# amcpherson/remixt

Hardware: AMD Instinct MI355X
Metric: EM iterations/sec (50k seg x 165 states) (higher is better)
Workload: dtype f64

## Files before the change

### include/remixt_amd.h

```cpp
#ifndef REMIXT_AMD_H
#define REMIXT_AMD_H

#include <stdint.h>

#ifdef __cplusplus
extern "C" {
#endif

#define RMX_OK 0
#define RMX_EVALUE 1
#define RMX_EASSERT 2
#define RMX_EDEVICE 3
#define RMX_EUNSUPPORTED 4
#define RMX_EARG 5

#define RMX_MAX_CLONES 4

typedef struct rmx_batch rmx_batch;

typedef struct rmx_problem {
    int32_t num_clones;
    int32_t num_segments;
    int32_t num_breakpoints;
    int32_t num_cn_states;
// ... 58 lines not shown
    RMX_OPT_SEARCH_MODE,
    RMX_OPT_ELL_DENSE,
    RMX_OPT_STRIP,
    RMX_OPT_CELL_CACHE,
    RMX_OPT_SPARSE_TRIAL,
    RMX_OPT_FB_DEBUG,
    RMX_OPT_PAIRWISE_KERNEL,
    RMX_OPT_PACE_SWEEPS,
    RMX_OPT_FB_WG_BUDGET,
    RMX_OPT_TRIAL_KERNEL,
    RMX_OPT_GRAD_KERNEL,
    RMX_OPT_STREAM_POOL,
    RMX_OPT_VITERBI_CLUSTER,
    RMX_OPT_TRACEBACK,
    RMX_OPT_LT_CLASSES,
    RMX_OPT_COUNT
};
int rmx_set_default_option(int32_t option_id, int32_t value);
int rmx_set_option(rmx_batch *b, int32_t option_id, int32_t value);
int rmx_get_option(rmx_batch *b, int32_t option_id, int32_t *value);

int rmx_set_param(rmx_batch *b, int32_t r, int32_t param_id, double value);
int rmx_get_param(rmx_batch *b, int32_t r, int32_t param_id, double *value);
int rmx_set_transition_model(rmx_batch *b, int32_t model);
int rmx_set_array(rmx_batch *b, int32_t r, int32_t array_id, const void *host_src);
int rmx_get_array(rmx_batch *b, int32_t r, int32_t array_id, void *host_dst);
int rmx_fetch_indicators(rmx_batch *b, int32_t r0, int32_t r1, const double **total, const double **allele);
int rmx_calculate_log_transmat(rmx_batch *b, int32_t r, double *dst);
int rmx_weighted_search(const double *p, int64_t n, const double *u, int32_t k, int64_t *out, int64_t *positive);
int rmx_weighted_sample_round(const double *w, int64_t n, int64_t stride, double norm, const double *u, int32_t k,
// ... 74 lines not shown
```

### remixt_amd/bpmodel.py

```python
import ctypes as C

import numpy as np

from . import _lib

_dp = C.POINTER(C.c_double)
_ip = C.POINTER(C.c_int64)
_i32p = C.POINTER(C.c_int32)

RMX_EVALUE, RMX_EASSERT, RMX_EDEVICE, RMX_EUNSUPPORTED, RMX_EARG = 1, 2, 3, 4, 5

MAX_CLONES = 4
PARAM_IDS = {
    'negbin_r_0': 0, 'negbin_r_1': 1, 'negbin_hdel_mu': 2, 'negbin_hdel_r_0': 3, 'negbin_hdel_r_1': 4,
    'betabin_M_0': 5, 'betabin_M_1': 6, 'betabin_loh_p': 7, 'betabin_loh_M_0': 8, 'betabin_loh_M_1': 9,
    'prior_outlier_total': 10, 'prior_outlier_allele': 11, 'divergence_weight': 12, 'hmm_log_norm_const': 13,
}
ARRAY_IDS = {
    'h': 0, 'p_breakpoint': 1, 'p_allele_swap': 2, 'p_outlier_total': 3, 'p_outlier_allele': 4,
    'posterior_marginals': 5, 'framelogprob': 6, 'total_likelihood_mask': 7, 'allele_likelihood_mask': 8,
    'log_transmat': 9, 'cached_log_transmat': 10, 'joint_posterior_marginals': 11, 'state_sequence': 12,
}
_WRITABLE = {'h', 'p_breakpoint', 'p_allele_swap', 'p_outlier_total', 'p_outlier_allele', 'posterior_marginals',
             'total_likelihood_mask', 'allele_likelihood_mask'}
_STATE_TABLES = {'cn_states_total': 0, 'num_alleles_subclonal': 1, 'is_hdel': 2, 'is_loh': 3}


OPTION_IDS = dict((n, i) for i, n in enumerate((
    'fb_kernel', 'fb_nv', 'fb_breakend_codes', 'fuse_sweeps', 'two_streams', 'viterbi_plain', 'search_mode', 'ell_dense', 'strip',
    'cell_cache', 'sparse_trial', 'fb_debug', 'pairwise_kernel', 'pace_sweeps', 'fb_wg_budget', 'trial_kernel', 'grad_kernel', 'stream_pool', 'viterbi_cluster', 'traceback', 'lt_classes')))


def set_default_option(name, value):
    lib = _lib.load()
    rc = lib.rmx_set_default_option(OPTION_IDS[name], int(value))
    if rc:
        _raise(lib, rc)


def last_error_restarts():
    lib = _lib.load()
    n = lib.rmx_last_error_restarts(None, 0)
    if n <= 0:
        return []
    buf = (C.c_int32 * n)()
# ... 791 lines not shown
```

### remixt_amd/csrc/rmx_api.hip

```cpp
#include <hip/hip_runtime.h>
#include <algorithm>
#include <cmath>
#include <limits>
#include <atomic>
#include <cstdio>
#include <cstring>
#include <functional>
#include <map>
#include <mutex>
#include <string>
#include <vector>
#include <chrono>
#include <cstdlib>
#include <condition_variable>
#include <memory>

#include "rmx_kernels.h"
#include "rmx_host.h"

static thread_local std::string g_err;
static thread_local std::vector<int32_t> g_err_restarts;
static int fail(int code, const std::string &msg) { g_err = msg; g_err_restarts.clear(); return code; }
static int fail_flagged(int code, const std::string &msg) { g_err = msg; return code; }
static inline long long now_ns() { return std::chrono::duration_cast<std::chrono::nanoseconds>(std::chrono::steady_clock::now().time_since_epoch()).count(); }
// ... 21 lines not shown
    StreamPool &p = g_stream_pool[dev & 15];
    std::lock_guard<std::mutex> lk(p.mu);
    std::vector<hipStream_t> &idle = p.idle[role];
    if (!idle.empty()) { *out = idle.front(); idle.erase(idle.begin()); return RMX_OK; }
    if (hipStreamCreateWithFlags(out, hipStreamNonBlocking) != hipSuccess) return RMX_EDEVICE;
    p.created[role]++;
    return RMX_OK;
}
static void pool_release(int dev, int role, hipStream_t s) {
    hipStreamSynchronize(s);
    StreamPool &p = g_stream_pool[dev & 15];
    std::lock_guard<std::mutex> lk(p.mu);
    p.idle[role].push_back(s);
}

static int g_opt_default[RMX_OPT_COUNT] = {0, 0, 1, 1, 1, 0, 5, 0, 1, 1, 1, 0, 0, 0, 0, 0, 0, 1, 0, 0, 1};
static std::mutex g_opt_mu;

struct rmx_batch {
    hipEvent_t ev_pace = nullptr;
    int opt[RMX_OPT_COUNT];
    int device = 0;
    hipStream_t stream = nullptr;
    hipStream_t stream2 = nullptr;
    hipEvent_t ev_fb = nullptr, ev_brk = nullptr;
    bool own_stream = false, pooled_stream = false, pooled_stream2 = false;
    Dev d{};
    int R = 0;
    std::vector<int64_t> cn_classes;
    std::vector<int32_t> seg_class, brk_idx, brk_orient, tclass, brk_slot, be_n;
    std::vector<int64_t> brk_states, is_telomere;
// ... 25 lines not shown
    int32_t *h_lists = nullptr;
    size_t h_lists_cap = 0;
    hipEvent_t ev_lists = nullptr;
    uint32_t *h_err = nullptr;
    int32_t *d_sample = nullptr;
    NmState *d_nm_state = nullptr;
    NmLayout nm_lay = {nullptr, nullptr, nullptr}; double *d_nm_partial = nullptr; size_t nm_partial_cap = 0;
    int32_t *d_msample = nullptr, *d_mcounts = nullptr;
    std::vector<int> msample_count;
    double *d_mpartial = nullptr; size_t mpartial_cap = 0;
    std::vector<std::vector<int64_t>> sample_cache; std::vector<int> sample_count;
    double *d_grid_out = nullptr;
    GradFlatLayout gf_lay = {nullptr, nullptr, nullptr, nullptr};
    std::vector<double> gf_sig;
    std::vector<long long> sample_epoch, sig_epoch;
    int32_t *gf_nblk_host = nullptr;
    bool gf_first = false;
    unsigned *d_done = nullptr;
    int32_t *d_rlist = nullptr, *d_counts = nullptr; RestartParams *d_rp_stage = nullptr; double *d_batch_out = nullptr;
    void *h_batch = nullptr;
    std::vector<int32_t> plain_list; int32_t *d_plain_list = nullptr; double *d_plain_jt = nullptr;
    int last_search_blocks = 0;
    unsigned *d_vflag = nullptr; int cluster_timeouts = 0;
    int last_viterbi_wgs = 1;
    int32_t *d_vit_special = nullptr; int n_vit_special = -1;
    double *h_elbo = nullptr; hipEvent_t ev_elbo = nullptr; bool elbo_pending = false, elbo_sync = false; int elbo_r0 = 0, elbo_r1 = 0;
    double *d_vrow = nullptr; size_t vrow_cap = 0;
    uint16_t *d_bp = nullptr; double *d_final = nullptr; int64_t *d_path = nullptr; double *d_logprob = nullptr;
    std::vector<int64_t> last_path; int vit_cap = 0; size_t bp_cap = 0;
    int16_t *d_samp = nullptr; size_t samp_cap = 0; uint64_t *d_seeds = nullptr; uint32_t *d_sflags = nullptr;
// ... 78 lines not shown
        return id == KID_FRAMELOGPROB || id == KID_FB || id == KID_MARGINALS || id == KID_PAIRWISE || id == KID_BRK_LUT ||
               id == KID_BRK_UPDATE || id == KID_OUTLIER_TOTAL || id == KID_OUTLIER_ALLELE || id == KID_ALLELE_SWAP;
    }
    ProfScope(rmx_batch *b_, int id_) : b(b_), id(id_) {
        on = b->prof == 1 || (b->prof == 2 && sweep_kernel(id));
        if (on) { a = get_event(b); e = get_event(b); hipEventRecord(a, b->stream); }
    }
    void restart(int id_) { id = id_; if (on) hipEventRecord(a, b->stream); }
    void cancel() { if (on) { b->ev_pool.push_back(a); b->ev_pool.push_back(e); on = false; } }
    ~ProfScope() {
        if (on) { hipEventRecord(e, b->stream); b->prof_pending.push_back({id, a, e}); if (b->prof_pending.size() > 8192) prof_collect(b); }
    }
};

static int translate_error(rmx_batch *b, int r, uint32_t v);
static int check_errors(rmx_batch *b, int r0, int r1) {
    uint32_t *e = b->h_err;
    HIPCHK(hipMemcpyAsync(e, b->d.err, sizeof(uint32_t) * b->R, hipMemcpyDeviceToHost, b->stream));
    HIPCHK(hipStreamSynchronize(b->stream));
    int first = -1;
    for (int r = r0; r < r1; r++) if (e[r]) { if (first < 0) { first = r; g_err_restarts.clear(); } g_err_restarts.push_back(r); }
    if (first < 0) return RMX_OK;
    HIPCHK(hipMemsetAsync(b->d.err + r0, 0, sizeof(uint32_t) * (size_t)(r1 - r0), b->stream));
    return translate_error(b, first, e[first]);
}
template <typename F> static int report_request_errors(rmx_batch *b, int n, const uint32_t *words, F restart_of) {
    int first = -1;
    for (int i = 0; i < n; i++) {
        if (!words[i]) continue;
        const int r = restart_of(i);
        if (first < 0) { first = i; g_err_restarts.clear(); }
        if (std::find(g_err_restarts.begin(), g_err_restarts.end(), r) == g_err_restarts.end()) {
            g_err_restarts.push_back(r);
// ... 850 lines not shown
    return RMX_OK;
}
int rmx_synchronize(rmx_batch *b) { BIND(b); HIPCHK(hipStreamSynchronize(b->stream)); return RMX_OK; }

int rmx_info(rmx_batch *b, int32_t what, int64_t *out) { BIND(b);
    switch (what) {
    case 0: *out = b->d.cn_max; break; case 1: *out = b->d.NC; break; case 2: *out = b->d.TC; break; case 3: *out = b->d.NBE; break;
    case 4: *out = b->d.SP; break; case 5: *out = b->fbv_rpt; break; case 6: *out = b->fbG.P; break; case 7: *out = b->fbG.NT; break;
    case 8: *out = b->fbG.BLK; break; case 9: *out = (int64_t)b->fbG_lds; break; case 10: *out = b->n_fast; break; case 11: *out = b->n_generic; break;
    case 60: *out = b->t_launch_ns; break; case 61: *out = b->t_wait_ns; break; case 62: *out = b->t_post_ns; break; case 63: *out = b->n_rounds; break;
    case 12: *out = b->last_fb_kernel; break; case 13: *out = b->last_fb_nv; break; case 14: *out = b->last_viterbi; break; case 15: *out = b->last_fb_nv_max; break;
    case 18: *out = b->last_viterbi_wgs; break; case 19: *out = b->last_traceback; break;
    case 64: *out = b->d.NT; break; case 65: *out = b->d.ltc ? 1 : 0; break;
    case 54: *out = b->cluster_timeouts; break;
    case 52: *out = b->last_search_blocks; break;
    case 16: { StreamPool &p_ = g_stream_pool[b->device & 15]; std::lock_guard<std::mutex> lk(p_.mu); *out = p_.created[0] + p_.created[1]; break; }
    case 17: { StreamPool &p_ = g_stream_pool[b->device & 15]; std::lock_guard<std::mutex> lk(p_.mu); *out = (int64_t)(p_.idle[0].size() + p_.idle[1].size()); break; }
    case 20: case 21: case 22: case 23: case 24: case 25: case 26: case 27: case 28: case 29: case 30: case 31: case 32: case 33: case 34: case 35: case 36: case 37: case 38: case 39:
    case 40: case 41: case 42: case 43: case 44: case 45: case 46: case 47: case 48: case 49: case 50: case 51:
        { if (!b->d_dbg) { *out = 0; break; } unsigned long long v[32]; HIPCHK(hipStreamSynchronize(b->stream)); HIPCHK(hipMemcpy(v, b->d_dbg, 256, hipMemcpyDeviceToHost)); *out = (int64_t)v[what - 20]; break; }
    default: return fail(RMX_EARG, "bad info id");
    }
    return RMX_OK;
}

static const int kParamComponents[RMX_P_HMM_LOG_NORM_CONST] = {CM_LT0, CM_LT1, CM_LT0 | CM_LT1, CM_LT0, CM_LT1, CM_LA0, CM_LA1, CM_LA0 | CM_LA1, CM_LA0, CM_LA1, 0, 0, 16};
int rmx_set_param(rmx_batch *b, int32_t r, int32_t id, double v) { BIND(b);
    if (r < 0 || r >= b->R || id < 0 || id >= RMX_P_HMM_LOG_NORM_CONST) return fail(RMX_EARG, "bad restart / param id");
    if (id == RMX_P_DIVERGENCE_WEIGHT) v = std::fabs(v);
    b->rp[r].p[id] = v; b->tables_dirty[r] = 1; b->ab_dirty[r] = 1;
// ... 604 lines not shown
    RANGE_CHECK();
    if (b->elbo_pending) return fail(RMX_EARG, "an ELBO is already pending: rmx_calculate_elbo_end first");
    const int nr = r1 - r0;
    if (!b->h_elbo) {
        HIPCHK(hipHostMalloc((void **)&b->h_elbo, ((size_t)b->R * 4 + (size_t)b->R) * 8, hipHostMallocDefault));
        HIPCHK(hipEventCreateWithFlags(&b->ev_elbo, hipEventDisableTiming));
    }
    bool mixed = false;
    for (int r = r0; r < r1; r++) mixed |= b->lt_valid[r] && b->lt_model[r] != b->cached_model[r];
    b->elbo_r0 = r0; b->elbo_r1 = r1; b->elbo_sync = mixed;
    b->elbo_pending = true;
    if (mixed) return RMX_OK;
    int rc = ensure_ab(b, r0, r1);
    if (rc) { b->elbo_pending = false; return rc; }
    { ProfScope ps(b, KID_ELBO_SEG); hipLaunchKernelGGL(k_elbo_seg, dim3(ELBO_BLOCKS, nr), dim3(256), 0, b->stream, b->d, r0, b->d_partial, b->d_be_e); }
    for (int r = r0; r < r1;) {
        int e = r + 1;
        while (e < r1 && b->plain_T_init[e] == b->plain_T_init[r]) e++;
        ProfScope ps(b, KID_ELBO_FINAL);
        hipLaunchKernelGGL(k_elbo_final, dim3(e - r), dim3(256), 0, b->stream, b->d, r, b->d_partial + (size_t)(r - r0) * ELBO_BLOCKS * 3,
                           b->d_be_e + (size_t)(r - r0) * b->d.NBE, ELBO_BLOCKS,
                           (const int *)b->d_lt_valid, b->plain_T_init[r], (const double *)nullptr, b->d_out4 + (size_t)(r - r0) * 4);
        r = e;
    }
    HIPCHK(hipGetLastError());
    HIPCHK(hipMemcpyAsync(b->h_elbo, b->d_out4, (size_t)nr * 32, hipMemcpyDeviceToHost, b->stream));
    HIPCHK(hipMemcpyAsync(b->h_elbo + (size_t)b->R * 4, b->d.err, sizeof(uint32_t) * b->R, hipMemcpyDeviceToHost, b->stream));
    HIPCHK(hipEventRecord(b->ev_elbo, b->stream));
    return RMX_OK;
}
int rmx_calculate_elbo_end(rmx_batch *b, double *out) { BIND(b);
    if (!b || !out) return fail(RMX_EARG, "bad argument");
    if (!b->elbo_pending) return fail(RMX_EARG, "no ELBO pending");
    b->elbo_pending = false;
    const int r0 = b->elbo_r0, r1 = b->elbo_r1;
    if (b->elbo_sync) return rmx_calculate_elbo(b, r0, r1, out);
    HIPCHK(hipEventSynchronize(b->ev_elbo));
    const uint32_t *e = reinterpret_cast<const uint32_t *>(b->h_elbo + (size_t)b->R * 4);
    int first = -1;
    for (int r = r0; r < r1; r++) if (e[r]) { if (first < 0) { first = r; g_err_restarts.clear(); } g_err_restarts.push_back(r); }
    if (first >= 0) {
        std::lock_guard<std::mutex> lk(b->mu);
// ... 113 lines not shown
        }
        HIPCHK(hipMemcpyAsync(hp, gout, (size_t)G * W * 8, hipMemcpyDeviceToHost, b->stream));
        if ((rc = finish_restart(b, r, eh))) return rc;
    }
    HIPCHK(hipEventSynchronize(b->done_ev[r]));
    if (*eh) { uint32_t v = *eh; std::lock_guard<std::mutex> lk(b->mu); HIPCHK(hipMemsetAsync(b->d.err + r, 0, sizeof(uint32_t), b->stream)); return translate_error(b, r, v); }
    for (int g = 0; g < G; g++) out[g] = hp[(size_t)g * W];
    return RMX_OK;
}

static bool gradflat_ready(rmx_batch *b, int nreq, const int32_t *restarts, const StageArgs &sa) {
    if (!b->gf_lay.upre) {
        const size_t R = (size_t)b->R;
        if (dalloc(b, &b->gf_lay.upre, R * (NM_MAX_SAMPLE + 1)) != RMX_OK || dalloc(b, &b->gf_lay.blk, R * (NM_MAX_SAMPLE + 2)) != RMX_OK ||
            dalloc(b, &b->gf_lay.nblk, R) != RMX_OK || dalloc(b, &b->gf_lay.k8, R * NM_MAX_SAMPLE * 8) != RMX_OK) { b->gf_lay.upre = nullptr; return false; }
        if (hipHostMalloc((void **)&b->gf_nblk_host, 16 * sizeof(int32_t), hipHostMallocDefault) != hipSuccess) { b->gf_lay.upre = nullptr; return false; }
    }
    std::vector<double> sig;
    sig.reserve((size_t)nreq * (3 + RMX_P_HMM_LOG_NORM_CONST));
    for (int i = 0; i < nreq; i++) {
        const int r = restarts[i];
        sig.push_back((double)r); sig.push_back((double)b->sample_epoch[r]); sig.push_back((double)b->sig_epoch[r]);
        for (int k = 0; k < RMX_P_HMM_LOG_NORM_CONST; k++) sig.push_back(sa.rp[i].p[k]);
    }
    if (sig == b->gf_sig) return true;
    hipLaunchKernelGGL(k_gradflat_setup, dim3(nreq), dim3(256), 0, b->stream, b->d, sa, (const int32_t *)b->d_sample, (const int32_t *)b->d_counts, b->gf_lay, b->gf_nblk_host);
    if (hipGetLastError() != hipSuccess) return false;
    b->gf_sig.swap(sig);
    b->gf_first = true;
    return true;
}
static int run_ell_batch(rmx_batch *b, int nreq, const int32_t *restarts, bool grad, double *out, int mask = CM_ALL) {
    const Dev &d = b->d;
    const long long t_in = now_ns();
    const int W = 1 + RMX_MAX_CLONES;
    const int nout = grad ? W : 1;
    int maxcnt = 0;
    const bool by_value = nreq <= 16;
    StageArgs sa;
    RestartParams *hs = by_value ? sa.rp : (RestartParams *)b->h_batch;
    int32_t *hl = by_value ? sa.rlist : (int32_t *)((char *)b->h_batch + (size_t)b->R * sizeof(RestartParams));
    for (int i = 0; i < nreq; i++) {
        const int r = restarts[i];
// ... 10 lines not shown
            ProfScope ps(b, KID_STATE_TABLES);
            hipLaunchKernelGGL(k_state_tables_list_v, dim3(d.C, nreq), dim3(256), 0, b->stream, b->d, sa, b->d_rlist, b->d_rp_stage);
        } else {
            HIPCHK(hipMemcpyAsync(b->d_rp_stage, hs, (size_t)nreq * sizeof(RestartParams), hipMemcpyHostToDevice, b->stream));
            HIPCHK(hipMemcpyAsync(b->d_rlist, hl, (size_t)nreq * 4, hipMemcpyHostToDevice, b->stream));
            ProfScope ps(b, KID_STATE_TABLES);
            hipLaunchKernelGGL(k_state_tables_list, dim3(d.C, nreq), dim3(256), 0, b->stream, b->d, (const int32_t *)b->d_rlist, (const RestartParams *)b->d_rp_stage);
        }
        const int pstride = std::max(d.N, ELBO_BLOCKS) * W;
        bool final_done = false;
        if (maxcnt > 0) {
            ProfScope ps(b, KID_ELL_LIST);
            if (grad && by_value && ell_sparse_ok(b, nreq, restarts) && b->opt[RMX_OPT_GRAD_KERNEL] == 0 && maxcnt <= NM_MAX_SAMPLE && gradflat_ready(b, nreq, restarts, sa)) {
                int nb = 0;
                if (b->gf_first) nb = (maxcnt * SEGL + 255) / 256 + 1;
                else for (int i = 0; i < nreq; i++) nb = std::max(nb, (int)b->gf_nblk_host[i]);
                b->gf_first = false;
                hipLaunchKernelGGL(k_gradflat_round, dim3(std::max(nb, 1), nreq), dim3(256), 0, b->stream, b->d, (const int32_t *)b->d_rlist, (const RestartParams *)b->d_rp_stage,
                                   (const int32_t *)b->d_sample, (const int32_t *)b->d_counts, b->gf_lay, b->d_ell_partial, pstride);
            }
            else if (grad && ell_sparse_ok(b, nreq, restarts) && b->opt[RMX_OPT_GRAD_KERNEL] != 1)
                hipLaunchKernelGGL(k_ell_list_batch_sparse_grad, dim3((maxcnt + SEG_PER_BLOCK - 1) / SEG_PER_BLOCK, nreq), dim3(256), 0, b->stream, b->d, (const int32_t *)b->d_rlist,
                                   (const RestartParams *)b->d_rp_stage, (const int32_t *)b->d_sample, (const int32_t *)b->d_counts, b->d_ell_partial, pstride);
            else if (grad && ell_sparse_ok(b, nreq, restarts)) {
                hipLaunchKernelGGL(k_ell_list_batch_sparse_grad_final, dim3((maxcnt + SEG_PER_BLOCK - 1) / SEG_PER_BLOCK, nreq), dim3(256), 0, b->stream, b->d, (const int32_t *)b->d_rlist,
                                   (const RestartParams *)b->d_rp_stage, (const int32_t *)b->d_sample, (const int32_t *)b->d_counts, b->d_ell_partial, pstride,
                                   b->d_done, res, nout, eres);
                final_done = true;
            }
            else if (grad) hipLaunchKernelGGL(k_ell_list_batch<true>, dim3(maxcnt, nreq), ell_block(b), 0, b->stream, b->d, (const int32_t *)b->d_rlist, (const RestartParams *)b->d_rp_stage,
                                         (const int32_t *)b->d_sample, (const int32_t *)b->d_counts, b->d_ell_partial, pstride);
// ... 389 lines not shown
int rmx_expected_ll_h_batch(rmx_batch *b, int32_t nreq, const int32_t *restarts, const double *h, double *out) { BIND(b);
    if (!b || nreq < 1 || nreq > b->R || !restarts || !h || !out) return fail(RMX_EARG, "bad argument");
    int rc = check_request_list(b, nreq, restarts);
    if (rc) return rc;
    for (int i = 0; i < nreq; i++)
        if ((rc = rmx_set_array(b, restarts[i], RMX_A_H, h + (size_t)i * b->d.M))) return rc;
    return run_ell_batch(b, nreq, restarts, true, out);
}

int rmx_expected_ll_full(rmx_batch *b, int32_t r0, int32_t r1, double *out) { BIND(b);
    RANGE_CHECK();
    int rc = ensure_ab(b, r0, r1);
    if (rc) return rc;
    const int nr = r1 - r0;
    { ProfScope ps(b, KID_ELL_FULL); hipLaunchKernelGGL(k_ell_full_batch, dim3(ELBO_BLOCKS, nr), dim3(256), 0, b->stream, b->d, r0, b->d_partial); }
    { ProfScope ps(b, KID_ELL_FINAL); hipLaunchKernelGGL(k_sum_partials, dim3(nr), dim3(256), 0, b->stream, (const double *)b->d_partial, ELBO_BLOCKS, b->d_out4); }
    HIPCHK(hipGetLastError());
    HIPCHK(hipMemcpyAsync(b->h_pinned, b->d_out4, (size_t)nr * 8, hipMemcpyDeviceToHost, b->stream));
    if ((rc = check_errors(b, r0, r1))) return rc;
    for (int i = 0; i < nr; i++) out[i] = b->h_pinned[i];
    return RMX_OK;
}

static int trial_pass(rmx_batch *b, int r0, int r1, Dev &d2) {
    b->trial_comp_r0 = b->trial_comp_r1 = -1;
    b->scratch_r0 = b->scratch_r1 = -1;
    int rc = ensure_tables(b, r0, r1);
    if (rc) return rc;
    const Dev &d = b->d;
    const int nr = r1 - r0;
    const size_t RN0 = (size_t)r0 * d.N, cnt = (size_t)nr * d.N;
    HIPCHK(hipMemcpyAsync(b->d_A2 + RN0 * 2, d.A + RN0 * 2, cnt * 16, hipMemcpyDeviceToDevice, b->stream));
    HIPCHK(hipMemcpyAsync(b->d_Bv2 + RN0 * 4, d.Bv + RN0 * 4, cnt * 32, hipMemcpyDeviceToDevice, b->stream));
    d2 = b->d;
    d2.A = b->d_A2; d2.Bv = b->d_Bv2; d2.lc = nullptr; d2.ltc = nullptr;
    for (int r = r0; r < r1;) {
        const int mask = use_strip(b) ? cover_mask(b->comp_dirty[r] & 15) : (b->comp_dirty[r] ? 15 : 0);
        int e = r + 1;
        while (e < r1 && (use_strip(b) ? cover_mask(b->comp_dirty[e] & 15) : (b->comp_dirty[e] ? 15 : 0)) == mask) e++;
        if (mask) {
            ProfScope ps(b, KID_MARGINALS_AB);
            bool sparse = use_strip(b) && d.sig_cnt != nullptr;
            for (int i = r; i < e; i++) if (!b->sig_valid[i]) sparse = false;
            if (sparse) {
                void (*kf)(Dev, int) = nullptr;
                if (b->opt[RMX_OPT_TRIAL_KERNEL] == 0) {
                    switch (mask) {
                    case 1: kf = k_trial_flat<1>; break; case 2: kf = k_trial_flat<2>; break; case 3: kf = k_trial_flat<3>; break;
                    case 4: kf = k_trial_flat<4>; break; case 8: kf = k_trial_flat<8>; break; case 12: kf = k_trial_flat<12>; break;
                    default: kf = k_trial_flat<15>; break;
                    }
                    hipLaunchKernelGGL(kf, dim3((d.N + TF_SEGB - 1) / TF_SEGB, e - r), dim3(256), 0, b->stream, d2, r);
                } else {
                    switch (mask) {
                    case 1: kf = k_trial_sparse<1>; break; case 2: kf = k_trial_sparse<2>; break; case 3: kf = k_trial_sparse<3>; break;
                    case 4: kf = k_trial_sparse<4>; break; case 8: kf = k_trial_sparse<8>; break; case 12: kf = k_trial_sparse<12>; break;
                    default: kf = k_trial_sparse<15>; break;
                    }
// ... 4 lines not shown
            else hipLaunchKernelGGL(k_marginals<false>, row_grid(b, e - r), dim3(256), 0, b->stream, d2, r, b->G);
        }
        r = e;
    }
    b->scratch_r0 = r0; b->scratch_r1 = r1;
    return RMX_OK;
}
int rmx_expected_ll_full_trial(rmx_batch *b, int32_t r0, int32_t r1, double *out) { BIND(b);
    RANGE_CHECK();
    Dev d2;
    int rc = trial_pass(b, r0, r1, d2);
    if (rc) return rc;
    const int nr = r1 - r0;
    double *cpart = b->d_partial + (size_t)b->R * ELBO_BLOCKS, *cout = b->d_out4 + b->R;
    b->trial_comp_r0 = b->trial_comp_r1 = -1;
    { ProfScope ps(b, KID_ELL_FULL); hipLaunchKernelGGL(k_ell_full_batch, dim3(ELBO_BLOCKS, nr), dim3(256), 0, b->stream, d2, r0, b->d_partial); }
    { ProfScope ps(b, KID_ELL_FINAL); hipLaunchKernelGGL(k_sum_partials, dim3(nr), dim3(256), 0, b->stream, (const double *)b->d_partial, ELBO_BLOCKS, b->d_out4); }
    { ProfScope ps(b, KID_ELL_FULL); hipLaunchKernelGGL(k_ell_comp_batch, dim3(ELBO_BLOCKS, nr), dim3(256), 0, b->stream, d2, r0, cpart); }
    { ProfScope ps(b, KID_ELL_FINAL); hipLaunchKernelGGL(k_sum_partials, dim3(nr * 4), dim3(256), 0, b->stream, (const double *)cpart, ELBO_BLOCKS, cout); }
    HIPCHK(hipGetLastError());
    HIPCHK(hipMemcpyAsync(b->h_pinned, b->d_out4, (size_t)nr * 8, hipMemcpyDeviceToHost, b->stream));
    HIPCHK(hipMemcpyAsync(b->h_pinned + nr, cout, (size_t)nr * 32, hipMemcpyDeviceToHost, b->stream));
    if ((rc = check_errors(b, r0, r1))) return rc;
    for (int i = 0; i < nr; i++) out[i] = b->h_pinned[i];
    b->trial_comp.assign(b->h_pinned + nr, b->h_pinned + nr + (size_t)nr * 4);
    b->trial_comp_r0 = r0; b->trial_comp_r1 = r1;
    return RMX_OK;
}
int rmx_expected_ll_components(rmx_batch *b, int32_t r0, int32_t r1, int32_t trial, double *out) { BIND(b);
    RANGE_CHECK();
    if (!out) return fail(RMX_EARG, "bad argument");
    int rc;
    Dev d2 = b->d;
    if (trial == 2 && b->trial_comp_r0 == r0 && b->trial_comp_r1 == r1) {
        for (int i = 0; i < (r1 - r0) * 4; i++) out[i] = b->trial_comp[i];
        return RMX_OK;
    }
    if (trial == 3) {
        if (b->trial_comp_r0 != r0 || b->trial_comp_r1 != r1) return fail(RMX_EUNSUPPORTED, "no trial pass over this range to take the expectations from");
        const int nr = r1 - r0;
        bool own = false;
        for (int r = r0; r < r1; r++) own |= b->comp_dirty[r] == 0;
        if (own) {
            { ProfScope ps(b, KID_ELL_FULL); hipLaunchKernelGGL(k_ell_comp_batch, dim3(ELBO_BLOCKS, nr), dim3(256), 0, b->stream, d2, r0, b->d_partial); }
            { ProfScope ps(b, KID_ELL_FINAL); hipLaunchKernelGGL(k_sum_partials, dim3(nr * 4), dim3(256), 0, b->stream, (const double *)b->d_partial, ELBO_BLOCKS, b->d_out4); }
            HIPCHK(hipGetLastError());
            HIPCHK(hipMemcpyAsync(b->h_pinned, b->d_out4, (size_t)nr * 32, hipMemcpyDeviceToHost, b->stream));
            if ((rc = check_errors(b, r0, r1))) return rc;
        }
        for (int r = r0; r < r1; r++)
            for (int c = 0; c < 4; c++) out[(r - r0) * 4 + c] = b->comp_dirty[r] != 0 ? b->trial_comp[(size_t)(r - r0) * 4 + c] : b->h_pinned[(r - r0) * 4 + c];
        return RMX_OK;
    }
    if (trial == 2) {
        if (b->scratch_r0 != r0 || b->scratch_r1 != r1) return fail(RMX_EUNSUPPORTED, "no trial pass over this range to take the expectations from");
        d2.A = b->d_A2; d2.Bv = b->d_Bv2;
    }
    else if (trial) { if ((rc = trial_pass(b, r0, r1, d2))) return rc; }
    else if ((rc = ensure_ab(b, r0, r1))) return rc;
    const int nr = r1 - r0;
    { ProfScope ps(b, KID_ELL_FULL); hipLaunchKernelGGL(k_ell_comp_batch, dim3(ELBO_BLOCKS, nr), dim3(256), 0, b->stream, d2, r0, b->d_partial); }
    { ProfScope ps(b, KID_ELL_FINAL); hipLaunchKernelGGL(k_sum_partials, dim3(nr * 4), dim3(256), 0, b->stream, (const double *)b->d_partial, ELBO_BLOCKS, b->d_out4); }
    HIPCHK(hipGetLastError());
    HIPCHK(hipMemcpyAsync(b->h_pinned, b->d_out4, (size_t)nr * 32, hipMemcpyDeviceToHost, b->stream));
    if ((rc = check_errors(b, r0, r1))) return rc;
    for (int i = 0; i < nr * 4; i++) out[i] = b->h_pinned[i];
    return RMX_OK;
}
int rmx_trial_rollback(rmx_batch *b, int32_t r, int32_t param_id, const double *values) { BIND(b);
    if (!b || r < 0 || r >= b->R || !values || param_id >= RMX_P_HMM_LOG_NORM_CONST) return fail(RMX_EARG, "bad argument");
    if (param_id >= 0) b->rp[r].p[param_id] = param_id == RMX_P_DIVERGENCE_WEIGHT ? std::fabs(values[0]) : values[0];
    else for (int m = 0; m < b->d.M; m++) b->rp[r].h[m] = values[m];
    b->tables_dirty[r] = 1; b->segc_dirty[r] = 1;
    if (param_id >= 0 && param_id < RMX_P_HMM_LOG_NORM_CONST) {
        const int back = kParamComponents[param_id] & ~b->comp_base[r];
        b->comp_dirty[r] &= ~back; b->cache_stale[r] &= ~(back & 15);
        b->ab_dirty[r] = b->comp_dirty[r] != 0;
    } else { b->ab_dirty[r] = 0; b->comp_dirty[r] = 0; b->comp_base[r] = 0; b->cache_stale[r] = 0; }
    return RMX_OK;
}
// ... 467 lines not shown
```

### remixt_amd/csrc/rmx_kernels.h

```cpp
#pragma once
#include "rmx_device.h"
#include "rmx_host.h"
#define SEGL 32
#define SEG_PER_BLOCK (256 / SEGL)
#define TRIAL_SEGL 16
#define RMX_CLUSTER_SPINS (1u << 22)
#define FBK_WKN 128
#define NM_MAX_SAMPLE 1024
#define TRIAL_SEG_PER_BLOCK (256 / TRIAL_SEGL)


__device__ __forceinline__ void state_tables_body(const Dev &d, int cls, int r, const RestartParams &rp) {
    __shared__ unsigned agg_sh;
    if (threadIdx.x == 0) agg_sh = 0u;
    __syncthreads();
    unsigned agg = 0u;
    for (int s = threadIdx.x; s < d.S; s += blockDim.x) {
        const int8_t *cn = d.cn + ((size_t)cls * d.S + s) * d.M * 2;
        const int8_t *tot = d.tot + ((size_t)cls * d.S + s) * d.M;
        double minor = 0., total = 0.;
        for (int m = 0; m < d.M; m++) {
            minor += rp.h[m] * (double)cn[m * 2 + 0];
            total += rp.h[m] * (double)tot[m];
        }
// ... 2537 lines not shown
        partial[((size_t)(r - r0) * gridDim.x + blockIdx.x) * 3 + 1] = ent;
        partial[((size_t)(r - r0) * gridDim.x + blockIdx.x) * 3 + 2] = z;
    }
    for (int slot = blockIdx.x * blockDim.x + threadIdx.x; slot < d.NBE; slot += gridDim.x * blockDim.x) {
        double e = 0.;
        if (d.tclass[d.be_n[slot]] >= 0) {
            const double *h = d.hist + ((size_t)r * d.NBE + slot) * d.M * d.D;
            const double *pc = d.pd_cached + ((size_t)r * d.NBE + slot) * d.M * d.D;
            for (int i = 0; i < d.M * d.D; i++) e += h[i] * (-d.pen * pc[i]);
            e += -d.pen * d.be_ja[(size_t)r * d.NBE + slot];
        }
        be_e[(size_t)(r - r0) * d.NBE + slot] = e;
    }
}
__global__ void k_elbo_final(Dev d, int r0, const double *partial, const double *be_e, int nblk, const int *lt_valid, double plain_T_init,
                             const double *full_plain, double *out) {
    __shared__ double scratch[8];
    const int r = r0 + blockIdx.x, t = threadIdx.x;
    double en = 0., ent = 0., z = 0.;
    if (t == 0) for (int i = 0; i < nblk; i++) {
        const double *pp = partial + ((size_t)blockIdx.x * nblk + i) * 3;
        en += pp[0]; ent += pp[1]; z += pp[2];
    }
    double hb = 0.;
    for (int i = t; i < d.K * d.B; i += 256) hb += xlogx(d.pbrk[(size_t)r * d.K * d.B + i]);
    hb = block_sum<256>(hb, scratch);
    double ec = 0., jt = 0.;
    for (int slot = t; slot < d.NBE; slot += 256) {
        if (d.tclass[d.be_n[slot]] < 0) continue;
        ec += be_e[(size_t)blockIdx.x * d.NBE + slot];
        jt += d.be_jt[(size_t)r * d.NBE + slot];
    }
    ec = block_sum<256>(ec, scratch);
// ... 248 lines not shown
        lay.k8[((size_t)r * NM_MAX_SAMPLE + i) * 8 + k] = seg_const_value(rp, x, y0, ys, k);
    }
    __syncthreads();
    if (threadIdx.x == 0) {
        int32_t *up = lay.upre + (size_t)r * (NM_MAX_SAMPLE + 1), *bl = lay.blk + (size_t)r * (NM_MAX_SAMPLE + 2);
        int a = 0, nb = 0, inblk = 0;
        up[0] = 0;
        if (cnt > 0) bl[nb++] = 0;
        for (int i = 0; i < cnt; i++) {
            const int u = un[i + 1];
            if (inblk + u > 256) { bl[nb++] = i; inblk = 0; }
            inblk += u; a += u; up[i + 1] = a;
        }
        bl[nb] = cnt;
        lay.nblk[r] = nb;
        nblk_host[blockIdx.x] = nb;
    }
}
__global__ __launch_bounds__(256) void k_gradflat_round(Dev d, const int32_t *rlist, const RestartParams *stage, const int32_t *samples, const int32_t *counts,
                                                        GradFlatLayout lay, double *partial, int pstride) {
    __shared__ int lpre[257];
    __shared__ double vals[1 + RMX_MAX_CLONES][256];
    const int r = rlist[blockIdx.y], tid = threadIdx.x;
    if ((int)blockIdx.x >= lay.nblk[r]) return;
    const RestartParams &rp = stage[blockIdx.y];
    const int32_t *bl = lay.blk + (size_t)r * (NM_MAX_SAMPLE + 2), *up = lay.upre + (size_t)r * (NM_MAX_SAMPLE + 1);
    const int i0 = bl[blockIdx.x], i1 = bl[blockIdx.x + 1], nseg = i1 - i0;
    const int u0 = up[i0];
    for (int k = tid; k <= nseg; k += 256) lpre[k] = up[i0 + k] - u0;
    __syncthreads();
    const int nunits = lpre[nseg];
// ... 351 lines not shown
    if (!go) {
        out[2 * req] = nm.xopt(); out[2 * req + 1] = last;
        done_out[req] = 1u + d.err[r];
    }
}
__global__ void k_ell_search_final(Dev d, SearchVals sv, const int32_t *counts, const double *partial, int maxcnt, double *out, uint32_t *err_out) {
    __shared__ double scratch[8];
    const int req = blockIdx.x / sv.Gz;
    const int r = sv.rlist[req];
    if (err_out && threadIdx.x == 0 && blockIdx.x % sv.Gz == 0) err_out[req] = d.err[r];
    double a = 0.;
    for (int i = threadIdx.x; i < counts[r]; i += 256) a += partial[(size_t)blockIdx.x * maxcnt + i];
    a = block_sum<256>(a, scratch);
    if (threadIdx.x == 0) out[blockIdx.x] = a;
}
__global__ void k_ell_full_batch(Dev d, int r0, double *partial) {
    __shared__ double scratch[8];
    const int r = r0 + blockIdx.y;
    double acc = 0.;
    for (int n = blockIdx.x * blockDim.x + threadIdx.x; n < d.N; n += gridDim.x * blockDim.x) {
        const size_t rn = (size_t)r * d.N + n;
        const double qt0 = d.qt[rn * 2], qt1 = d.qt[rn * 2 + 1], qa0 = d.qa[rn * 2], qa1 = d.qa[rn * 2 + 1];
        const double qs0 = d.qs[rn * 2], qs1 = d.qs[rn * 2 + 1];
        acc += qt0 * d.A[rn * 2] + qt1 * d.A[rn * 2 + 1];
        acc += qa0 * qs0 * d.Bv[rn * 4] + qa0 * qs1 * d.Bv[rn * 4 + 1] + qa1 * qs0 * d.Bv[rn * 4 + 2] + qa1 * qs1 * d.Bv[rn * 4 + 3];
    }
    acc = block_sum<256>(acc, scratch);
    if (threadIdx.x == 0) partial[(size_t)blockIdx.y * gridDim.x + blockIdx.x] = acc;
}
__global__ void k_ell_comp_batch(Dev d, int r0, double *partial) {
    __shared__ double scratch[8];
    const int r = r0 + blockIdx.y;
    double c0 = 0., c1 = 0., c2 = 0., c3 = 0.;
    for (int n = blockIdx.x * blockDim.x + threadIdx.x; n < d.N; n += gridDim.x * blockDim.x) {
        const size_t rn = (size_t)r * d.N + n;
        const double qt0 = d.qt[rn * 2], qt1 = d.qt[rn * 2 + 1], qa0 = d.qa[rn * 2], qa1 = d.qa[rn * 2 + 1];
        const double qs0 = d.qs[rn * 2], qs1 = d.qs[rn * 2 + 1];
        c0 += qt0 * d.A[rn * 2]; c1 += qt1 * d.A[rn * 2 + 1];
        c2 += qa0 * qs0 * d.Bv[rn * 4] + qa0 * qs1 * d.Bv[rn * 4 + 1];
        c3 += qa1 * qs0 * d.Bv[rn * 4 + 2] + qa1 * qs1 * d.Bv[rn * 4 + 3];
    }
    c0 = block_sum<256>(c0, scratch); c1 = block_sum<256>(c1, scratch); c2 = block_sum<256>(c2, scratch); c3 = block_sum<256>(c3, scratch);
    if (threadIdx.x == 0) {
        double *pp = partial + (size_t)blockIdx.y * 4 * gridDim.x + blockIdx.x;
        pp[0] = c0; pp[gridDim.x] = c1; pp[2 * gridDim.x] = c2; pp[3 * gridDim.x] = c3;
    }
}
__global__ void k_sum_partials(const double *partial, int n, double *out) {
    __shared__ double scratch[8];
    double a = 0.;
    for (int i = threadIdx.x; i < n; i += 256) a += partial[(size_t)blockIdx.x * n + i];
    a = block_sum<256>(a, scratch);
    if (threadIdx.x == 0) out[blockIdx.x] = a;
}

__global__ void k_logz(Dev d, int r, double *out) {
    __shared__ double scratch[8];
    double z = 0.;
    for (int n = threadIdx.x; n < d.N; n += 256) z += d.rowZ[(size_t)r * d.N + n];
    z = block_sum<256>(z, scratch);
    if (threadIdx.x == 0) *out = z;
}

__global__ void k_cell_probe(Dev d, int r, int n, int s, double *out6) {
// ... 1816 lines not shown
```

Before: 452.3.

## Write reductions directly to pinned host memory and skip redundant trial copies and setups

Adds three options, all on by default. The first skips the device-to-device A/Bv copy for trial restart groups that are fully recomputed sparsely. The second has the final reduction kernels write results and error flags straight into pinned host buffers, which removes the follow-up memcpy calls and fuses the full and component ELL sums into one kernel. The third reruns grad-flat setup only for restarts whose signature changed, with the per-restart nblk host buffer indexed by restart. This cuts copies and launches on the EM path, but relies on kernel writes to host memory being visible after stream sync, and adds per-restart bookkeeping.

```diff
diff --git a/include/remixt_amd.h b/include/remixt_amd.h
--- a/include/remixt_amd.h
+++ b/include/remixt_amd.h
@@ -96,6 +96,9 @@
     RMX_OPT_VITERBI_CLUSTER,
     RMX_OPT_TRACEBACK,
     RMX_OPT_LT_CLASSES,
+    RMX_OPT_TRIAL_NOCOPY,
+    RMX_OPT_ELL_DIRECT,
+    RMX_OPT_GRADFLAT_SETUP,
     RMX_OPT_COUNT
 };
 int rmx_set_default_option(int32_t option_id, int32_t value);
diff --git a/remixt_amd/bpmodel.py b/remixt_amd/bpmodel.py
--- a/remixt_amd/bpmodel.py
+++ b/remixt_amd/bpmodel.py
@@ -28,7 +28,8 @@
 
 OPTION_IDS = dict((n, i) for i, n in enumerate((
     'fb_kernel', 'fb_nv', 'fb_breakend_codes', 'fuse_sweeps', 'two_streams', 'viterbi_plain', 'search_mode', 'ell_dense', 'strip',
-    'cell_cache', 'sparse_trial', 'fb_debug', 'pairwise_kernel', 'pace_sweeps', 'fb_wg_budget', 'trial_kernel', 'grad_kernel', 'stream_pool', 'viterbi_cluster', 'traceback', 'lt_classes')))
+    'cell_cache', 'sparse_trial', 'fb_debug', 'pairwise_kernel', 'pace_sweeps', 'fb_wg_budget', 'trial_kernel', 'grad_kernel', 'stream_pool', 'viterbi_cluster', 'traceback', 'lt_classes',
+    'trial_nocopy', 'ell_direct', 'gradflat_setup')))
 
 
 def set_default_option(name, value):
diff --git a/remixt_amd/csrc/rmx_api.hip b/remixt_amd/csrc/rmx_api.hip
--- a/remixt_amd/csrc/rmx_api.hip
+++ b/remixt_amd/csrc/rmx_api.hip
@@ -59,7 +59,7 @@
     p.idle[role].push_back(s);
 }
 
-static int g_opt_default[RMX_OPT_COUNT] = {0, 0, 1, 1, 1, 0, 5, 0, 1, 1, 1, 0, 0, 0, 0, 0, 0, 1, 0, 0, 1};
+static int g_opt_default[RMX_OPT_COUNT] = {0, 0, 1, 1, 1, 0, 5, 0, 1, 1, 1, 0, 0, 0, 0, 0, 0, 1, 0, 0, 1, 1, 1, 1};
 static std::mutex g_opt_mu;
 
 struct rmx_batch {
@@ -115,6 +115,8 @@
     GradFlatLayout gf_lay = {nullptr, nullptr, nullptr, nullptr};
     std::vector<double> gf_sig;
     std::vector<long long> sample_epoch, sig_epoch;
+    std::vector<double> gf_rsig; std::vector<char> gf_rsig_set;
+    long long gf_setups = 0;
     int32_t *gf_nblk_host = nullptr;
     bool gf_first = false;
     unsigned *d_done = nullptr;
@@ -223,9 +225,9 @@
 };
 
 static int translate_error(rmx_batch *b, int r, uint32_t v);
-static int check_errors(rmx_batch *b, int r0, int r1) {
+static int check_errors(rmx_batch *b, int r0, int r1, bool landed = false) {
     uint32_t *e = b->h_err;
-    HIPCHK(hipMemcpyAsync(e, b->d.err, sizeof(uint32_t) * b->R, hipMemcpyDeviceToHost, b->stream));
+    if (!landed) HIPCHK(hipMemcpyAsync(e, b->d.err, sizeof(uint32_t) * b->R, hipMemcpyDeviceToHost, b->stream));
     HIPCHK(hipStreamSynchronize(b->stream));
     int first = -1;
     for (int r = r0; r < r1; r++) if (e[r]) { if (first < 0) { first = r; g_err_restarts.clear(); } g_err_restarts.push_back(r); }
@@ -1106,6 +1108,7 @@
     case 64: *out = b->d.NT; break; case 65: *out = b->d.ltc ? 1 : 0; break;
     case 54: *out = b->cluster_timeouts; break;
     case 52: *out = b->last_search_blocks; break;
+    case 55: *out = b->gf_setups; break;
     case 16: { StreamPool &p_ = g_stream_pool[b->device & 15]; std::lock_guard<std::mutex> lk(p_.mu); *out = p_.created[0] + p_.created[1]; break; }
     case 17: { StreamPool &p_ = g_stream_pool[b->device & 15]; std::lock_guard<std::mutex> lk(p_.mu); *out = (int64_t)(p_.idle[0].size() + p_.idle[1].size()); break; }
     case 20: case 21: case 22: case 23: case 24: case 25: case 26: case 27: case 28: case 29: case 30: case 31: case 32: case 33: case 34: case 35: case 36: case 37: case 38: case 39:
@@ -1740,18 +1743,22 @@
     int rc = ensure_ab(b, r0, r1);
     if (rc) { b->elbo_pending = false; return rc; }
     { ProfScope ps(b, KID_ELBO_SEG); hipLaunchKernelGGL(k_elbo_seg, dim3(ELBO_BLOCKS, nr), dim3(256), 0, b->stream, b->d, r0, b->d_partial, b->d_be_e); }
+    const bool direct = b->opt[RMX_OPT_ELL_DIRECT] != 0;
     for (int r = r0; r < r1;) {
         int e = r + 1;
         while (e < r1 && b->plain_T_init[e] == b->plain_T_init[r]) e++;
         ProfScope ps(b, KID_ELBO_FINAL);
         hipLaunchKernelGGL(k_elbo_final, dim3(e - r), dim3(256), 0, b->stream, b->d, r, b->d_partial + (size_t)(r - r0) * ELBO_BLOCKS * 3,
                            b->d_be_e + (size_t)(r - r0) * b->d.NBE, ELBO_BLOCKS,
-                           (const int *)b->d_lt_valid, b->plain_T_init[r], (const double *)nullptr, b->d_out4 + (size_t)(r - r0) * 4);
+                           (const int *)b->d_lt_valid, b->plain_T_init[r], (const double *)nullptr, (direct ? b->h_elbo : b->d_out4) + (size_t)(r - r0) * 4,
+                           direct ? reinterpret_cast<uint32_t *>(b->h_elbo + (size_t)b->R * 4) : (uint32_t *)nullptr);
         r = e;
     }
     HIPCHK(hipGetLastError());
-    HIPCHK(hipMemcpyAsync(b->h_elbo, b->d_out4, (size_t)nr * 32, hipMemcpyDeviceToHost, b->stream));
-    HIPCHK(hipMemcpyAsync(b->h_elbo + (size_t)b->R * 4, b->d.err, sizeof(uint32_t) * b->R, hipMemcpyDeviceToHost, b->stream));
+    if (!direct) {
+        HIPCHK(hipMemcpyAsync(b->h_elbo, b->d_out4, (size_t)nr * 32, hipMemcpyDeviceToHost, b->stream));
+        HIPCHK(hipMemcpyAsync(b->h_elbo + (size_t)b->R * 4, b->d.err, sizeof(uint32_t) * b->R, hipMemcpyDeviceToHost, b->stream));
+    }
     HIPCHK(hipEventRecord(b->ev_elbo, b->stream));
     return RMX_OK;
 }
@@ -1895,7 +1902,7 @@
         const size_t R = (size_t)b->R;
         if (dalloc(b, &b->gf_lay.upre, R * (NM_MAX_SAMPLE + 1)) != RMX_OK || dalloc(b, &b->gf_lay.blk, R * (NM_MAX_SAMPLE + 2)) != RMX_OK ||
             dalloc(b, &b->gf_lay.nblk, R) != RMX_OK || dalloc(b, &b->gf_lay.k8, R * NM_MAX_SAMPLE * 8) != RMX_OK) { b->gf_lay.upre = nullptr; return false; }
-        if (hipHostMalloc((void **)&b->gf_nblk_host, 16 * sizeof(int32_t), hipHostMallocDefault) != hipSuccess) { b->gf_lay.upre = nullptr; return false; }
+        if (hipHostMalloc((void **)&b->gf_nblk_host, R * sizeof(int32_t), hipHostMallocDefault) != hipSuccess) { b->gf_lay.upre = nullptr; return false; }
     }
     std::vector<double> sig;
     sig.reserve((size_t)nreq * (3 + RMX_P_HMM_LOG_NORM_CONST));
@@ -1904,10 +1911,25 @@
         sig.push_back((double)r); sig.push_back((double)b->sample_epoch[r]); sig.push_back((double)b->sig_epoch[r]);
         for (int k = 0; k < RMX_P_HMM_LOG_NORM_CONST; k++) sig.push_back(sa.rp[i].p[k]);
     }
-    if (sig == b->gf_sig) return true;
-    hipLaunchKernelGGL(k_gradflat_setup, dim3(nreq), dim3(256), 0, b->stream, b->d, sa, (const int32_t *)b->d_sample, (const int32_t *)b->d_counts, b->gf_lay, b->gf_nblk_host);
-    if (hipGetLastError() != hipSuccess) return false;
-    b->gf_sig.swap(sig);
+    const int SW = 2 + RMX_P_HMM_LOG_NORM_CONST;
+    if (b->gf_rsig.size() != (size_t)b->R * SW) { b->gf_rsig.assign((size_t)b->R * SW, 0.); b->gf_rsig_set.assign((size_t)b->R, 0); }
+    StageArgs sub;
+    int nsub = 0;
+    const bool per_list = b->opt[RMX_OPT_GRADFLAT_SETUP] == 0, all = per_list && sig != b->gf_sig;
+    for (int i = 0; i < nreq; i++) {
+        const int r = restarts[i];
+        const double *si = sig.data() + (size_t)i * (SW + 1) + 1;
+        double *sr = b->gf_rsig.data() + (size_t)r * SW;
+        if (!all && (per_list || (b->gf_rsig_set[r] && std::equal(si, si + SW, sr)))) continue;
+        std::copy(si, si + SW, sr); b->gf_rsig_set[r] = 1;
+        sub.rlist[nsub] = r; sub.rp[nsub] = sa.rp[i]; nsub++;
+    }
+    if (per_list) b->gf_sig.swap(sig); else b->gf_sig.clear();
+    if (nsub == 0) return true;
+    for (int i = nsub; i < 16; i++) { sub.rlist[i] = sub.rlist[0]; sub.rp[i] = sub.rp[0]; }
+    hipLaunchKernelGGL(k_gradflat_setup, dim3(nsub), dim3(256), 0, b->stream, b->d, sub, (const int32_t *)b->d_sample, (const int32_t *)b->d_counts, b->gf_lay, b->gf_nblk_host);
+    if (hipGetLastError() != hipSuccess) { for (int i = 0; i < nsub; i++) b->gf_rsig_set[sub.rlist[i]] = 0; b->gf_sig.clear(); return false; }
+    b->gf_setups++;
     b->gf_first = true;
     return true;
 }
@@ -1948,7 +1970,7 @@
             if (grad && by_value && ell_sparse_ok(b, nreq, restarts) && b->opt[RMX_OPT_GRAD_KERNEL] == 0 && maxcnt <= NM_MAX_SAMPLE && gradflat_ready(b, nreq, restarts, sa)) {
                 int nb = 0;
                 if (b->gf_first) nb = (maxcnt * SEGL + 255) / 256 + 1;
-                else for (int i = 0; i < nreq; i++) nb = std::max(nb, (int)b->gf_nblk_host[i]);
+                else for (int i = 0; i < nreq; i++) nb = std::max(nb, (int)b->gf_nblk_host[restarts[i]]);
                 b->gf_first = false;
                 hipLaunchKernelGGL(k_gradflat_round, dim3(std::max(nb, 1), nreq), dim3(256), 0, b->stream, b->d, (const int32_t *)b->d_rlist, (const RestartParams *)b->d_rp_stage,
                                    (const int32_t *)b->d_sample, (const int32_t *)b->d_counts, b->gf_lay, b->d_ell_partial, pstride);
@@ -2368,10 +2390,13 @@
     if (rc) return rc;
     const int nr = r1 - r0;
     { ProfScope ps(b, KID_ELL_FULL); hipLaunchKernelGGL(k_ell_full_batch, dim3(ELBO_BLOCKS, nr), dim3(256), 0, b->stream, b->d, r0, b->d_partial); }
-    { ProfScope ps(b, KID_ELL_FINAL); hipLaunchKernelGGL(k_sum_partials, dim3(nr), dim3(256), 0, b->stream, (const double *)b->d_partial, ELBO_BLOCKS, b->d_out4); }
+    const bool direct = b->opt[RMX_OPT_ELL_DIRECT] != 0;
+    { ProfScope ps(b, KID_ELL_FINAL);
+      if (direct) hipLaunchKernelGGL(k_sum_partials_host, dim3(nr), dim3(256), 0, b->stream, b->d, (const double *)b->d_partial, ELBO_BLOCKS, b->h_pinned, r0, nr, b->h_err);
+      else hipLaunchKernelGGL(k_sum_partials, dim3(nr), dim3(256), 0, b->stream, (const double *)b->d_partial, ELBO_BLOCKS, b->d_out4); }
     HIPCHK(hipGetLastError());
-    HIPCHK(hipMemcpyAsync(b->h_pinned, b->d_out4, (size_t)nr * 8, hipMemcpyDeviceToHost, b->stream));
-    if ((rc = check_errors(b, r0, r1))) return rc;
+    if (!direct) HIPCHK(hipMemcpyAsync(b->h_pinned, b->d_out4, (size_t)nr * 8, hipMemcpyDeviceToHost, b->stream));
+    if ((rc = check_errors(b, r0, r1, direct))) return rc;
     for (int i = 0; i < nr; i++) out[i] = b->h_pinned[i];
     return RMX_OK;
 }
@@ -2382,20 +2407,25 @@
     int rc = ensure_tables(b, r0, r1);
     if (rc) return rc;
     const Dev &d = b->d;
-    const int nr = r1 - r0;
-    const size_t RN0 = (size_t)r0 * d.N, cnt = (size_t)nr * d.N;
-    HIPCHK(hipMemcpyAsync(b->d_A2 + RN0 * 2, d.A + RN0 * 2, cnt * 16, hipMemcpyDeviceToDevice, b->stream));
-    HIPCHK(hipMemcpyAsync(b->d_Bv2 + RN0 * 4, d.Bv + RN0 * 4, cnt * 32, hipMemcpyDeviceToDevice, b->stream));
+    const bool copy_all = b->opt[RMX_OPT_TRIAL_NOCOPY] == 0;
+    auto copy_own = [&](int ra, int rb) -> int {
+        const size_t o = (size_t)ra * d.N, c = (size_t)(rb - ra) * d.N;
+        HIPCHK(hipMemcpyAsync(b->d_A2 + o * 2, d.A + o * 2, c * 16, hipMemcpyDeviceToDevice, b->stream));
+        HIPCHK(hipMemcpyAsync(b->d_Bv2 + o * 4, d.Bv + o * 4, c * 32, hipMemcpyDeviceToDevice, b->stream));
+        return RMX_OK;
+    };
+    if (copy_all && (rc = copy_own(r0, r1))) return rc;
     d2 = b->d;
     d2.A = b->d_A2; d2.Bv = b->d_Bv2; d2.lc = nullptr; d2.ltc = nullptr;
     for (int r = r0; r < r1;) {
         const int mask = use_strip(b) ? cover_mask(b->comp_dirty[r] & 15) : (b->comp_dirty[r] ? 15 : 0);
         int e = r + 1;
         while (e < r1 && (use_strip(b) ? cover_mask(b->comp_dirty[e] & 15) : (b->comp_dirty[e] ? 15 : 0)) == mask) e++;
+        bool sparse = use_strip(b) && d.sig_cnt != nullptr;
+        for (int i = r; i < e; i++) if (!b->sig_valid[i]) sparse = false;
+        if (!copy_all && !(mask == 15 && sparse) && (rc = copy_own(r, e))) return rc;
         if (mask) {
             ProfScope ps(b, KID_MARGINALS_AB);
-            bool sparse = use_strip(b) && d.sig_cnt != nullptr;
-            for (int i = r; i < e; i++) if (!b->sig_valid[i]) sparse = false;
             if (sparse) {
                 void (*kf)(Dev, int) = nullptr;
                 if (b->opt[RMX_OPT_TRIAL_KERNEL] == 0) {
@@ -2430,6 +2460,17 @@
     const int nr = r1 - r0;
     double *cpart = b->d_partial + (size_t)b->R * ELBO_BLOCKS, *cout = b->d_out4 + b->R;
     b->trial_comp_r0 = b->trial_comp_r1 = -1;
+    if (b->opt[RMX_OPT_ELL_DIRECT]) {
+        { ProfScope ps(b, KID_ELL_FULL); hipLaunchKernelGGL(k_ell_full_comp_batch, dim3(ELBO_BLOCKS, nr), dim3(256), 0, b->stream, d2, r0, b->d_partial); }
+        { ProfScope ps(b, KID_ELL_FINAL); hipLaunchKernelGGL(k_sum_partials_host, dim3(nr * 5), dim3(256), 0, b->stream, b->d, (const double *)b->d_partial, ELBO_BLOCKS,
+                                                             b->h_pinned, r0, nr, b->h_err); }
+        HIPCHK(hipGetLastError());
+        if ((rc = check_errors(b, r0, r1, true))) return rc;
+        for (int i = 0; i < nr; i++) out[i] = b->h_pinned[i];
+        b->trial_comp.assign(b->h_pinned + nr, b->h_pinned + nr + (size_t)nr * 4);
+        b->trial_comp_r0 = r0; b->trial_comp_r1 = r1;
+        return RMX_OK;
+    }
     { ProfScope ps(b, KID_ELL_FULL); hipLaunchKernelGGL(k_ell_full_batch, dim3(ELBO_BLOCKS, nr), dim3(256), 0, b->stream, d2, r0, b->d_partial); }
     { ProfScope ps(b, KID_ELL_FINAL); hipLaunchKernelGGL(k_sum_partials, dim3(nr), dim3(256), 0, b->stream, (const double *)b->d_partial, ELBO_BLOCKS, b->d_out4); }
     { ProfScope ps(b, KID_ELL_FULL); hipLaunchKernelGGL(k_ell_comp_batch, dim3(ELBO_BLOCKS, nr), dim3(256), 0, b->stream, d2, r0, cpart); }
@@ -2443,6 +2484,17 @@
     b->trial_comp_r0 = r0; b->trial_comp_r1 = r1;
     return RMX_OK;
 }
+static int comp_sums(rmx_batch *b, const Dev &dv, int r0, int r1) {
+    const int nr = r1 - r0;
+    const bool direct = b->opt[RMX_OPT_ELL_DIRECT] != 0;
+    { ProfScope ps(b, KID_ELL_FULL); hipLaunchKernelGGL(k_ell_comp_batch, dim3(ELBO_BLOCKS, nr), dim3(256), 0, b->stream, dv, r0, b->d_partial); }
+    { ProfScope ps(b, KID_ELL_FINAL);
+      if (direct) hipLaunchKernelGGL(k_sum_partials_host, dim3(nr * 4), dim3(256), 0, b->stream, b->d, (const double *)b->d_partial, ELBO_BLOCKS, b->h_pinned, r0, nr, b->h_err);
+      else hipLaunchKernelGGL(k_sum_partials, dim3(nr * 4), dim3(256), 0, b->stream, (const double *)b->d_partial, ELBO_BLOCKS, b->d_out4); }
+    HIPCHK(hipGetLastError());
+    if (!direct) HIPCHK(hipMemcpyAsync(b->h_pinned, b->d_out4, (size_t)nr * 32, hipMemcpyDeviceToHost, b->stream));
+    return check_errors(b, r0, r1, direct);
+}
 int rmx_expected_ll_components(rmx_batch *b, int32_t r0, int32_t r1, int32_t trial, double *out) { BIND(b);
     RANGE_CHECK();
     if (!out) return fail(RMX_EARG, "bad argument");
@@ -2457,13 +2509,7 @@
         const int nr = r1 - r0;
         bool own = false;
         for (int r = r0; r < r1; r++) own |= b->comp_dirty[r] == 0;
-        if (own) {
-            { ProfScope ps(b, KID_ELL_FULL); hipLaunchKernelGGL(k_ell_comp_batch, dim3(ELBO_BLOCKS, nr), dim3(256), 0, b->stream, d2, r0, b->d_partial); }
-            { ProfScope ps(b, KID_ELL_FINAL); hipLaunchKernelGGL(k_sum_partials, dim3(nr * 4), dim3(256), 0, b->stream, (const double *)b->d_partial, ELBO_BLOCKS, b->d_out4); }
-            HIPCHK(hipGetLastError());
-            HIPCHK(hipMemcpyAsync(b->h_pinned, b->d_out4, (size_t)nr * 32, hipMemcpyDeviceToHost, b->stream));
-            if ((rc = check_errors(b, r0, r1))) return rc;
-        }
+        if (own && (rc = comp_sums(b, d2, r0, r1))) return rc;
         for (int r = r0; r < r1; r++)
             for (int c = 0; c < 4; c++) out[(r - r0) * 4 + c] = b->comp_dirty[r] != 0 ? b->trial_comp[(size_t)(r - r0) * 4 + c] : b->h_pinned[(r - r0) * 4 + c];
         return RMX_OK;
@@ -2475,11 +2521,7 @@
     else if (trial) { if ((rc = trial_pass(b, r0, r1, d2))) return rc; }
     else if ((rc = ensure_ab(b, r0, r1))) return rc;
     const int nr = r1 - r0;
-    { ProfScope ps(b, KID_ELL_FULL); hipLaunchKernelGGL(k_ell_comp_batch, dim3(ELBO_BLOCKS, nr), dim3(256), 0, b->stream, d2, r0, b->d_partial); }
-    { ProfScope ps(b, KID_ELL_FINAL); hipLaunchKernelGGL(k_sum_partials, dim3(nr * 4), dim3(256), 0, b->stream, (const double *)b->d_partial, ELBO_BLOCKS, b->d_out4); }
-    HIPCHK(hipGetLastError());
-    HIPCHK(hipMemcpyAsync(b->h_pinned, b->d_out4, (size_t)nr * 32, hipMemcpyDeviceToHost, b->stream));
-    if ((rc = check_errors(b, r0, r1))) return rc;
+    if ((rc = comp_sums(b, d2, r0, r1))) return rc;
     for (int i = 0; i < nr * 4; i++) out[i] = b->h_pinned[i];
     return RMX_OK;
 }
diff --git a/remixt_amd/csrc/rmx_kernels.h b/remixt_amd/csrc/rmx_kernels.h
--- a/remixt_amd/csrc/rmx_kernels.h
+++ b/remixt_amd/csrc/rmx_kernels.h
@@ -2575,9 +2575,10 @@
     }
 }
 __global__ void k_elbo_final(Dev d, int r0, const double *partial, const double *be_e, int nblk, const int *lt_valid, double plain_T_init,
-                             const double *full_plain, double *out) {
+                             const double *full_plain, double *out, uint32_t *err_out = nullptr) {
     __shared__ double scratch[8];
     const int r = r0 + blockIdx.x, t = threadIdx.x;
+    if (err_out && t == 0) err_out[r] = d.err[r];
     double en = 0., ent = 0., z = 0.;
     if (t == 0) for (int i = 0; i < nblk; i++) {
         const double *pp = partial + ((size_t)blockIdx.x * nblk + i) * 3;
@@ -2856,7 +2857,7 @@
         }
         bl[nb] = cnt;
         lay.nblk[r] = nb;
-        nblk_host[blockIdx.x] = nb;
+        nblk_host[r] = nb;
     }
 }
 __global__ __launch_bounds__(256) void k_gradflat_round(Dev d, const int32_t *rlist, const RestartParams *stage, const int32_t *samples, const int32_t *counts,
@@ -3238,9 +3239,7 @@
     a = block_sum<256>(a, scratch);
     if (threadIdx.x == 0) out[blockIdx.x] = a;
 }
-__global__ void k_ell_full_batch(Dev d, int r0, double *partial) {
-    __shared__ double scratch[8];
-    const int r = r0 + blockIdx.y;
+__device__ __forceinline__ double ell_full_block(const Dev &d, int r, double *scratch) {
     double acc = 0.;
     for (int n = blockIdx.x * blockDim.x + threadIdx.x; n < d.N; n += gridDim.x * blockDim.x) {
         const size_t rn = (size_t)r * d.N + n;
@@ -3249,12 +3248,9 @@
         acc += qt0 * d.A[rn * 2] + qt1 * d.A[rn * 2 + 1];
         acc += qa0 * qs0 * d.Bv[rn * 4] + qa0 * qs1 * d.Bv[rn * 4 + 1] + qa1 * qs0 * d.Bv[rn * 4 + 2] + qa1 * qs1 * d.Bv[rn * 4 + 3];
     }
-    acc = block_sum<256>(acc, scratch);
-    if (threadIdx.x == 0) partial[(size_t)blockIdx.y * gridDim.x + blockIdx.x] = acc;
-}
-__global__ void k_ell_comp_batch(Dev d, int r0, double *partial) {
-    __shared__ double scratch[8];
-    const int r = r0 + blockIdx.y;
+    return block_sum<256>(acc, scratch);
+}
+__device__ __forceinline__ void ell_comp_block(const Dev &d, int r, double *scratch, double *pp, size_t pitch) {
     double c0 = 0., c1 = 0., c2 = 0., c3 = 0.;
     for (int n = blockIdx.x * blockDim.x + threadIdx.x; n < d.N; n += gridDim.x * blockDim.x) {
         const size_t rn = (size_t)r * d.N + n;
@@ -3265,13 +3261,33 @@
         c3 += qa1 * qs0 * d.Bv[rn * 4 + 2] + qa1 * qs1 * d.Bv[rn * 4 + 3];
     }
     c0 = block_sum<256>(c0, scratch); c1 = block_sum<256>(c1, scratch); c2 = block_sum<256>(c2, scratch); c3 = block_sum<256>(c3, scratch);
-    if (threadIdx.x == 0) {
-        double *pp = partial + (size_t)blockIdx.y * 4 * gridDim.x + blockIdx.x;
-        pp[0] = c0; pp[gridDim.x] = c1; pp[2 * gridDim.x] = c2; pp[3 * gridDim.x] = c3;
-    }
+    if (threadIdx.x == 0) { pp[0] = c0; pp[pitch] = c1; pp[2 * pitch] = c2; pp[3 * pitch] = c3; }
+}
+__global__ void k_ell_full_batch(Dev d, int r0, double *partial) {
+    __shared__ double scratch[8];
+    const double acc = ell_full_block(d, r0 + blockIdx.y, scratch);
+    if (threadIdx.x == 0) partial[(size_t)blockIdx.y * gridDim.x + blockIdx.x] = acc;
+}
+__global__ void k_ell_comp_batch(Dev d, int r0, double *partial) {
+    __shared__ double scratch[8];
+    ell_comp_block(d, r0 + blockIdx.y, scratch, partial + (size_t)blockIdx.y * 4 * gridDim.x + blockIdx.x, gridDim.x);
+}
+__global__ void k_ell_full_comp_batch(Dev d, int r0, double *partial) {
+    __shared__ double scratch[8];
+    const double acc = ell_full_block(d, r0 + blockIdx.y, scratch);
+    if (threadIdx.x == 0) partial[(size_t)blockIdx.y * gridDim.x + blockIdx.x] = acc;
+    ell_comp_block(d, r0 + blockIdx.y, scratch, partial + ((size_t)gridDim.y + (size_t)blockIdx.y * 4) * gridDim.x + blockIdx.x, gridDim.x);
 }
 __global__ void k_sum_partials(const double *partial, int n, double *out) {
     __shared__ double scratch[8];
+    double a = 0.;
+    for (int i = threadIdx.x; i < n; i += 256) a += partial[(size_t)blockIdx.x * n + i];
+    a = block_sum<256>(a, scratch);
+    if (threadIdx.x == 0) out[blockIdx.x] = a;
+}
+__global__ void k_sum_partials_host(Dev d, const double *partial, int n, double *out, int r0, int nr, uint32_t *err_out) {
+    __shared__ double scratch[8];
+    if ((int)blockIdx.x < nr && threadIdx.x == 0) err_out[r0 + blockIdx.x] = d.err[r0 + blockIdx.x];
     double a = 0.;
     for (int i = threadIdx.x; i < n; i += 256) a += partial[(size_t)blockIdx.x * n + i];
     a = block_sum<256>(a, scratch);
```

Result: no change. 456.2 (median of 4 runs) (+0.9%).
